# wavey-ai/soundkit

Measured on AMD Instinct MI355X. Metric: AAC-LC 1024-sample frames/s (whole node) + xrealtime, batch=4096 48 kHz stereo, higher is better.
Workload: dtype f32 (synthesis f32; s16 between the kernels as in the reference; FIR: the 16-bit samples as 2 x f16 exactly, the f32 taps as 2 x f16 to 2^-24, f32 accumulate; 1.0e-7 rel. RMS vs f64)

## Files before the change

soundkit_amd/csrc/aac_synth.hip:

```cpp
#include "sk_device.h"

#define SK_SYNTH_LOAD(p) (*(p))
#define SK_SYNTH_STORE(v, p) (*(p) = (v))

namespace sk {

namespace {

typedef float f2 __attribute__((ext_vector_type(2)));
typedef float f4 __attribute__((ext_vector_type(4)));

#ifndef SK_SYNTH_BLOCK_WAVES
#define SK_SYNTH_BLOCK_WAVES 4
#endif
constexpr int kWavesPerBlock = SK_SYNTH_BLOCK_WAVES;
#ifndef SK_WAVES_PER_SIMD
#define SK_WAVES_PER_SIMD 3
#endif
#ifndef SK_PREFETCH_DEPTH
#define SK_PREFETCH_DEPTH 1
#endif
constexpr int kDepth = SK_PREFETCH_DEPTH;
constexpr int kWavesPerSimd = SK_WAVES_PER_SIMD;
constexpr int kExchange = 576;
constexpr int kStage = 1024;

__device__ __forceinline__ f2 cmul(f2 a, f2 b) {
    return (f2){fmaf(a.x, b.x, -a.y * b.y), fmaf(a.x, b.y, a.y * b.x)};
}
__device__ __forceinline__ f2 cadd(f2 a, f2 b) { return (f2){a.x + b.x, a.y + b.y}; }
__device__ __forceinline__ f2 csub(f2 a, f2 b) { return (f2){a.x - b.x, a.y - b.y}; }
__device__ __forceinline__ f2 mul_mi(f2 a) { return (f2){a.y, -a.x}; }

__device__ __forceinline__ void dft8(f2 (&x)[8]) {
    const float h = 0.70710678118654752440f;
    f2 t0 = cadd(x[0], x[4]), t1 = csub(x[0], x[4]);
    f2 t2 = cadd(x[2], x[6]), t3 = mul_mi(csub(x[2], x[6]));
    f2 e0 = cadd(t0, t2), e2 = csub(t0, t2), e1 = cadd(t1, t3), e3 = csub(t1, t3);
    f2 u0 = cadd(x[1], x[5]), u1 = csub(x[1], x[5]);
    f2 u2 = cadd(x[3], x[7]), u3 = mul_mi(csub(x[3], x[7]));
    f2 o0 = cadd(u0, u2), o2 = csub(u0, u2), o1 = cadd(u1, u3), o3 = csub(u1, u3);
    f2 w1 = (f2){(o1.x + o1.y) * h, (o1.y - o1.x) * h};
    f2 w2 = mul_mi(o2);
    f2 w3 = (f2){(o3.y - o3.x) * h, -(o3.x + o3.y) * h};
    x[0] = cadd(e0, o0); x[4] = csub(e0, o0);
    x[1] = cadd(e1, w1); x[5] = csub(e1, w1);
    x[2] = cadd(e2, w2); x[6] = csub(e2, w2);
    x[3] = cadd(e3, w3); x[7] = csub(e3, w3);
}

__device__ __forceinline__ void wave_sync() {
    __builtin_amdgcn_fence(__ATOMIC_ACQ_REL, "wavefront");
    __builtin_amdgcn_wave_barrier();
}

typedef const __attribute__((address_space(4))) SynthEntry *const_entries;
__device__ __forceinline__ const_entries as_constant(const SynthEntry *p) {
    return reinterpret_cast<const_entries>(reinterpret_cast<uintptr_t>(p));
}

typedef uint32_t u2 __attribute__((ext_vector_type(2)));
__device__ __forceinline__ u2 pack4_s16(const f4 &v) {
    return (u2){dev_pack2_s16(v.x, v.y), dev_pack2_s16(v.z, v.w)};
}

__device__ __forceinline__ const float *first_half_window(const float *win, int seq, int prev_shape) {
    return seq == 3 ? win + 6656 + 1024 * prev_shape : win + 2048 * prev_shape;
}
__device__ __forceinline__ const float *second_half_window(const float *win, int seq, int shape) {
    return seq == 1 ? win + 4608 + 1024 * shape : win + 2048 * shape + 1024;
}

typedef __attribute__((address_space(3))) f2 lds_f2;
typedef __attribute__((address_space(3))) f4 lds_f4;
typedef __attribute__((address_space(3))) float lds_f;

__device__ __forceinline__ void read_positions(const lds_f *buf, int lane, float (&v)[16]) {
#pragma unroll
    for (int r = 0; r < 2; ++r) {
        const int j = 4 * lane + 256 * r;
        const f4 f = *reinterpret_cast<const lds_f4 *>(buf + j);
        const f4 m = *reinterpret_cast<const lds_f4 *>(buf + 1020 - j);
        v[8 * r + 0] = f.x; v[8 * r + 1] = f.y; v[8 * r + 2] = f.z; v[8 * r + 3] = f.w;
        v[8 * r + 4] = m.x; v[8 * r + 5] = m.y; v[8 * r + 6] = m.z; v[8 * r + 7] = m.w;
    }
}

__device__ __forceinline__ void write_positions(lds_f *buf, int lane, const float (&v)[16]) {
#pragma unroll
    for (int r = 0; r < 2; ++r) {
        const int j = 4 * lane + 256 * r;
        *reinterpret_cast<lds_f4 *>(buf + j) = (f4){v[8 * r + 0], v[8 * r + 1], v[8 * r + 2], v[8 * r + 3]};
        *reinterpret_cast<lds_f4 *>(buf + 1020 - j) = (f4){v[8 * r + 4], v[8 * r + 5], v[8 * r + 6], v[8 * r + 7]};
    }
}

__device__ __forceinline__ void fft512(f2 (&z)[8], lds_f2 *ex, const lds_f2 *t64, f2 base2, int lane) {
    const int hi3 = lane >> 3, lo3 = lane & 7;
    dft8(z);
#pragma unroll
    for (int k = 1; k < 8; ++k) z[k] = cmul(z[k], t64[8 * k + hi3]);
#pragma unroll
    for (int k = 0; k < 8; ++k) ex[k * 68 + lane] = z[k];
    wave_sync();
#pragma unroll
    for (int n2 = 0; n2 < 8; ++n2) z[n2] = cmul(ex[lo3 * 68 + 8 * n2 + hi3], base2);
    wave_sync();
    dft8(z);
#pragma unroll
    for (int k = 1; k < 8; ++k) z[k] = cmul(z[k], t64[8 * k + hi3]);
#pragma unroll
    for (int k = 0; k < 8; ++k) ex[hi3 * 72 + k * 8 + lo3] = z[k];
    wave_sync();
#pragma unroll
    for (int n3 = 0; n3 < 8; ++n3) z[n3] = ex[n3 * 72 + lane];
    wave_sync();
    dft8(z);
}

__device__ __attribute__((noinline)) void synth_rare_frame(lds_f2 *ex, lds_f *stage, const lds_f2 *tw_lds,
                                                            const lds_f2 *t64, float base2_re, float base2_im,
                                                            const lds_f *short_win, const lds_f2 *w64, const lds_f2 *tw_short,
                                                            float *out_ptr, int16_t *out16_ptr, int seq, int prev_shape,
                                                            int shape, int lane) {
    const int hi3 = lane >> 3, lo3 = lane & 7;
    (void)base2_re, (void)base2_im, (void)t64, (void)tw_lds, (void)seq;
    const lds_f *prev_short = short_win + 256 * prev_shape;
    const lds_f *cur_short = short_win + 256 * shape;
    f2 z[8];
#pragma unroll
    for (int r = 0; r < 8; ++r) z[r] = ex[64 * r + lane];
    float dly[16];
    read_positions(stage, lane, dly);
    wave_sync();
    float o[16], d[16];

    {
#pragma unroll
        for (int w = 0; w < 8; ++w) ex[64 * w + lane] = z[w];
        wave_sync();
#pragma unroll
        for (int b2 = 0; b2 < 8; ++b2) z[b2] = ex[64 * hi3 + lo3 + 8 * b2];
        wave_sync();
        dft8(z);
#pragma unroll
        for (int kb = 1; kb < 8; ++kb) z[kb] = cmul(z[kb], w64[lo3 * kb]);
#pragma unroll
        for (int kb = 0; kb < 8; ++kb) ex[64 * hi3 + 8 * kb + lo3] = z[kb];
        wave_sync();
#pragma unroll
        for (int aa = 0; aa < 8; ++aa) z[aa] = ex[64 * hi3 + 8 * lo3 + aa];
        wave_sync();
        dft8(z);
#pragma unroll
        for (int ka = 0; ka < 8; ++ka) {
            const int k = lo3 + 8 * ka;
            ex[64 * hi3 + k] = cmul(tw_short[k], (f2){z[ka].x, -z[ka].y});
        }
        wave_sync();
        const bool odd_lane = lane & 1;
        const int lo = odd_lane ? (63 - lane) >> 1 : lane >> 1;
        float cw[4], pw[2];
#pragma unroll
        for (int m = 0; m < 4; ++m) cw[m] = cur_short[lane + 64 * m];
        pw[0] = prev_short[lane];
        pw[1] = prev_short[lane + 64];
        float smp[8][4];
#pragma unroll
        for (int w = 0; w < 8; ++w) {
            const f2 A = ex[64 * w + lo], B = ex[64 * w + 32 + lo];
            const float s0 = odd_lane ? -A.y : -B.x, s1 = odd_lane ? B.x : A.y, s2 = odd_lane ? A.x : B.y, s3 = odd_lane ? B.y : A.x;
            smp[w][0] = s0 * (w == 0 ? pw[0] : cw[0]);
            smp[w][1] = s1 * (w == 0 ? pw[1] : cw[1]);
            smp[w][2] = s2 * cw[2];
            smp[w][3] = s3 * cw[3];
        }
        wave_sync();
#pragma unroll
        for (int half = 0; half < 2; ++half) {
#pragma unroll
            for (int r = 0; r < 4; ++r) *reinterpret_cast<lds_f4 *>(stage + 4 * lane + 256 * r) = (f4){0.f, 0.f, 0.f, 0.f};
            wave_sync();
#pragma unroll
            for (int parity = 0; parity < 2; ++parity) {
#pragma unroll
                for (int w = parity; w < 8; w += 2)
#pragma unroll
                    for (int m = 0; m < 4; ++m) {
                        const int base = 448 + 128 * w + 64 * m;
                        if ((base >> 10) != half) continue;
                        lds_f *at = stage + (base & 1023) + lane;
                        *at = *at + smp[w][m];
                    }
                wave_sync();
            }
            if (half == 0) read_positions(stage, lane, o);
            else read_positions(stage, lane, d);
            wave_sync();
        }
    }

    float pcm[16];
#pragma unroll
    for (int i = 0; i < 16; ++i) pcm[i] = o[i] + dly[i];
    write_positions((lds_f *)ex, lane, pcm);
    write_positions(stage, lane, d);
    wave_sync();
    (void)out_ptr, (void)out16_ptr;
}

template <bool OUT16, bool ONLY_LONG>
__global__ __launch_bounds__(kWavesPerBlock * 64, (ONLY_LONG && kDepth == 1) ? kWavesPerSimd + 1 : kWavesPerSimd) void k_aac_synth(SynthArgs a) {
    __shared__ f2 lds[kWavesPerBlock][kExchange];
    __shared__ float stage_lds[ONLY_LONG ? 1 : kWavesPerBlock][ONLY_LONG ? 4 : kStage];
    __shared__ f2 tw_tab[512];
    __shared__ f2 t64_tab[64];
    __shared__ float short_win_tab[ONLY_LONG ? 2 : 512];
    __shared__ f2 short_tw_tab[ONLY_LONG ? 1 : 128];

    const int lane = threadIdx.x & 63;
    const int wave = __builtin_amdgcn_readfirstlane(threadIdx.x >> 6);
    for (int i = threadIdx.x; i < 512; i += kWavesPerBlock * 64) tw_tab[i] = reinterpret_cast<const f2 *>(a.t.tw_long)[i];
    if (threadIdx.x < 64) t64_tab[threadIdx.x] = reinterpret_cast<const f2 *>(a.t.w64)[((threadIdx.x >> 3) * (threadIdx.x & 7)) & 63];
    if (!ONLY_LONG) {
        for (int i = threadIdx.x; i < 512; i += kWavesPerBlock * 64) short_win_tab[i] = a.t.win[4096 + i];
        if (threadIdx.x < 128)
            short_tw_tab[threadIdx.x] = threadIdx.x < 64 ? reinterpret_cast<const f2 *>(a.t.w64)[threadIdx.x] : reinterpret_cast<const f2 *>(a.t.tw_short)[threadIdx.x - 64];
    }
    __syncthreads();

    const uint32_t task_id = blockIdx.x * kWavesPerBlock + wave;
    if (task_id >= a.n_tasks) return;
    lds_f2 *ex = (lds_f2 *)lds[wave];
    lds_f *stage = (lds_f *)stage_lds[ONLY_LONG ? 0 : wave];
    const lds_f2 *tw_lds = (const lds_f2 *)tw_tab;
    const lds_f2 *t64 = (const lds_f2 *)t64_tab;

    const SynthTask task_v = a.tasks[task_id];
    const uint32_t count = __builtin_amdgcn_readfirstlane(task_v.count);
    const uint32_t state = __builtin_amdgcn_readfirstlane(task_v.state);
    if (count == 0) return;
    const const_entries entries = as_constant(a.entries + __builtin_amdgcn_readfirstlane(task_v.begin));

    const int hi3 = lane >> 3, lo3 = lane & 7;
    const f2 base2 = reinterpret_cast<const f2 *>(a.t.w512)[hi3 * lo3];

    float *delay_ptr = a.delay + (size_t)state * 1024;
    int prev_shape = __builtin_amdgcn_readfirstlane((int)a.prev_shape[state]);
    float dly[16];
    {
#pragma unroll
        for (int r = 0; r < 2; ++r) {
            const int j = 4 * lane + 256 * r;
            const f4 f = *reinterpret_cast<const f4 *>(delay_ptr + j);
            const f4 m = *reinterpret_cast<const f4 *>(delay_ptr + 1020 - j);
            dly[8 * r + 0] = f.x; dly[8 * r + 1] = f.y; dly[8 * r + 2] = f.z; dly[8 * r + 3] = f.w;
            dly[8 * r + 4] = m.x; dly[8 * r + 5] = m.y; dly[8 * r + 6] = m.z; dly[8 * r + 7] = m.w;
        }
    }

    auto load_spectrum = [&](f2 (&xin)[8], uint32_t e) {
        const float *src = a.coeffs + (size_t)__builtin_amdgcn_readfirstlane(entries[e].off1024) * 1024 + 2 * lane;
#pragma unroll
        for (int r = 0; r < 8; ++r) xin[r] = SK_SYNTH_LOAD(reinterpret_cast<const f2 *>(src + 128 * r));
    };
    auto frame = [&](f2 (&xin)[8], uint32_t e) __attribute__((always_inline)) {
        const uint32_t ent_off = entries[e].off1024, ent_win = entries[e].win;
        const uint32_t win = __builtin_amdgcn_readfirstlane(ent_win);
        const int seq = (int)(win & 3);
        const int shape = (win >> 2) & 1;
// ... 367 lines not shown
        }
        f4 f, m;
        f.x = -F0.x * W1f.x + dly[8 * r + 0]; f.y = -M1.y * W1f.y + dly[8 * r + 1];
        f.z = -F1.x * W1f.z + dly[8 * r + 2]; f.w = -M0.y * W1f.w + dly[8 * r + 3];
        m.x = M0.y * W1m.x + dly[8 * r + 4]; m.y = F1.x * W1m.y + dly[8 * r + 5];
        m.z = M1.y * W1m.z + dly[8 * r + 6]; m.w = F0.x * W1m.w + dly[8 * r + 7];
        if (OUT16) {
            SK_SYNTH_STORE(pack4_s16(f), reinterpret_cast<u2 *>(out16_ptr + j));
            SK_SYNTH_STORE(pack4_s16(m), reinterpret_cast<u2 *>(out16_ptr + 1020 - j));
        } else {
            SK_SYNTH_STORE(f, reinterpret_cast<f4 *>(out_ptr + j));
            SK_SYNTH_STORE(m, reinterpret_cast<f4 *>(out_ptr + 1020 - j));
        }
        dly[8 * r + 0] = F0.y * W2f.x; dly[8 * r + 1] = M1.x * W2f.y;
        dly[8 * r + 2] = F1.y * W2f.z; dly[8 * r + 3] = M0.x * W2f.w;
        dly[8 * r + 4] = M0.x * W2m.x; dly[8 * r + 5] = F1.y * W2m.y;
        dly[8 * r + 6] = M1.x * W2m.z; dly[8 * r + 7] = F0.y * W2m.w;
    };

    lds_f2 *stage = (lds_f2 *)stage_lds[WITH_SHORT ? wave : 0];
    auto store_pcm = [&](const float (&pcm)[16], uint32_t off) __attribute__((always_inline)) {
#pragma unroll
        for (int r = 0; r < 2; ++r) {
            const int j = 4 * lane + 256 * r;
            const f4 f = (f4){pcm[8 * r + 0], pcm[8 * r + 1], pcm[8 * r + 2], pcm[8 * r + 3]};
            const f4 m = (f4){pcm[8 * r + 4], pcm[8 * r + 5], pcm[8 * r + 6], pcm[8 * r + 7]};
            if (OUT16) {
                SK_SYNTH_STORE(pack4_s16(f), reinterpret_cast<u2 *>(a.pcm16 + (size_t)off * 1024 + j));
                SK_SYNTH_STORE(pack4_s16(m), reinterpret_cast<u2 *>(a.pcm16 + (size_t)off * 1024 + 1020 - j));
            } else {
                SK_SYNTH_STORE(f, reinterpret_cast<f4 *>(a.pcm + (size_t)off * 1024 + j));
                SK_SYNTH_STORE(m, reinterpret_cast<f4 *>(a.pcm + (size_t)off * 1024 + 1020 - j));
            }
        }
    };

    f2 xa[8], xb[8];
    load_spectrum(xa, ent_a, 0);
    load_spectrum(xb, ent_b, 0);
    for (uint32_t e = 0; e < count; ++e) {
        const uint32_t off_a = __builtin_amdgcn_readfirstlane(ent_a[e].off1024), off_b = __builtin_amdgcn_readfirstlane(ent_b[e].off1024);
        const uint32_t win_a = __builtin_amdgcn_readfirstlane(ent_a[e].win), win_b = __builtin_amdgcn_readfirstlane(ent_b[e].win);
        const int shape_a = (win_a >> 2) & 1, shape_b = (win_b >> 2) & 1;
        if constexpr (WITH_SHORT) {
            if ((win_a & 3u) == 2u) {
                {
                    const f2 tws = short_tw_tab[64 + lane];
                    const f2 tx = splat(tws.x), ty = splat(tws.y);
#pragma unroll
                    for (int w = 0; w < 8; ++w) {
                        const f2 even = (f2){xa[w].x, xb[w].x};
                        const f2 odd = (f2){-__shfl(xa[w].y, 63 - lane), -__shfl(xb[w].y, 63 - lane)};
                        const c2 zw = {odd * ty - even * tx, odd * tx + even * ty};
                        ex[64 * w + lane] = as_slot(zw);
                    }
                    f2 both[16];
#pragma unroll
                    for (int i = 0; i < 16; ++i) both[i] = (f2){dly_a[i], dly_b[i]};
                    write_positions2(stage, lane, both);
                    wave_sync();
                }
                synth_rare_pair(ex, stage, (const lds_f *)short_win_tab, (const lds_f2 *)short_tw_tab, (const lds_f2 *)short_tw_tab + 64, prev_a, shape_a, prev_b,
                                shape_b, lane);
                float pcm_a[16], pcm_b[16];
                {
                    f2 both[16];
                    read_positions2(stage, lane, both);
#pragma unroll
                    for (int i = 0; i < 16; ++i) {
                        dly_a[i] = both[i].x;
                        dly_b[i] = both[i].y;
                    }
                    read_positions2((const lds_f2 *)ex, lane, both);
#pragma unroll
                    for (int i = 0; i < 16; ++i) {
                        pcm_a[i] = both[i].x;
                        pcm_b[i] = both[i].y;
                    }
                    wave_sync();
                }
                const uint32_t ahead = e + 1 < count ? e + 1 : count - 1;
                load_spectrum(xa, ent_a, ahead);
                load_spectrum(xb, ent_b, ahead);
                store_pcm(pcm_a, off_a);
                store_pcm(pcm_b, off_b);
                prev_a = shape_a;
                prev_b = shape_b;
                continue;
            }
        }
        c2 z[8];
#pragma unroll
        for (int r = 0; r < 8; ++r) {
            const f2 even = (f2){xa[r].x, xb[r].x};
            const f2 odd = (f2){-__shfl(xa[7 - r].y, 63 - lane), -__shfl(xb[7 - r].y, 63 - lane)};
            const f2 t = tw_lds[lane + 64 * r];
            const f2 tx = splat(t.x), ty = splat(t.y);
            z[r] = {odd * ty - even * tx, odd * tx + even * ty};
        }
        Win wa, wb;
        int w1_a = 0, w2_a = 0, w1_b = 0, w2_b = 0;
        if constexpr (LDS_WIN) {
            const int seq_a = (int)(win_a & 3), seq_b = (int)(win_b & 3);
            w1_a = seq_a == 3 ? 6144 + 1024 * prev_a : 2048 * prev_a, w2_a = seq_a == 1 ? 4096 + 1024 * shape_a : 2048 * shape_a + 1024;
            w1_b = seq_b == 3 ? 6144 + 1024 * prev_b : 2048 * prev_b, w2_b = seq_b == 1 ? 4096 + 1024 * shape_b : 2048 * shape_b + 1024;
        } else {
            load_windows(wa, (int)(win_a & 3), prev_a, shape_a);
            load_windows(wb, (int)(win_b & 3), prev_b, shape_b);
        }
        {
            const uint32_t ahead = e + 1 < count ? e + 1 : count - 1;
            load_spectrum(xa, ent_a, ahead);
            load_spectrum(xb, ent_b, ahead);
        }
        fft512(z, ex, t64, base2, lane);
#pragma unroll
        for (int j = 0; j < 8; ++j) {
            const f2 t = tw_lds[lane + 64 * j];
            const f2 tx = splat(t.x), ty = splat(t.y);
            const c2 v = {fma2(tx, z[j].re, -(ty * -z[j].im)), fma2(tx, -z[j].im, ty * z[j].re)};
            ex[lane + 64 * j] = as_slot(v);
        }
        wave_sync();
        float *out_a = OUT16 ? nullptr : a.pcm + (size_t)off_a * 1024, *out_b = OUT16 ? nullptr : a.pcm + (size_t)off_b * 1024;
        int16_t *out16_a = OUT16 ? a.pcm16 + (size_t)off_a * 1024 : nullptr, *out16_b = OUT16 ? a.pcm16 + (size_t)off_b * 1024 : nullptr;
#pragma unroll
        for (int r = 0; r < 2; ++r) {
            const int q = 2 * lane + 128 * r;
            const f4 F0 = ex[256 + q], F1 = ex[257 + q], M0 = ex[254 - q], M1 = ex[255 - q];
            emit(r, (f2){F0.x, F0.z}, (f2){F1.x, F1.z}, (f2){M0.x, M0.z}, (f2){M1.x, M1.z}, wa, w1_a, w2_a, dly_a, out_a, out16_a);
            emit(r, (f2){F0.y, F0.w}, (f2){F1.y, F1.w}, (f2){M0.y, M0.w}, (f2){M1.y, M1.w}, wb, w1_b, w2_b, dly_b, out_b, out16_b);
        }
        wave_sync();
        prev_a = shape_a;
        prev_b = shape_b;
    }
    auto store_state = [&](float *p, const float (&d)[16]) {
#pragma unroll
        for (int r = 0; r < 2; ++r) {
            const int j = 4 * lane + 256 * r;
            *reinterpret_cast<f4 *>(p + j) = (f4){d[8 * r + 0], d[8 * r + 1], d[8 * r + 2], d[8 * r + 3]};
            *reinterpret_cast<f4 *>(p + 1020 - j) = (f4){d[8 * r + 4], d[8 * r + 5], d[8 * r + 6], d[8 * r + 7]};
        }
    };
    store_state(delay_a, dly_a);
    store_state(delay_b, dly_b);
    if (lane == 0) {
        a.prev_shape[state_a] = (uint8_t)prev_a;
        a.prev_shape[state_b] = (uint8_t)prev_b;
    }
}

constexpr int kTailRing = 2048;
constexpr int kTailDepth = 2;

__global__ __launch_bounds__(128, 2) void k_aac_tail(TailArgs ta) {
    const SynthArgs &a = ta.s;
    __shared__ f2 lds[2][kExchange];
    __shared__ f2 tw_tab[512];
    __shared__ f2 t64_tab[64];
    __shared__ __attribute__((aligned(16))) uint16_t ring_lds[2][2][kTailRing];
    __shared__ __attribute__((aligned(16))) uint32_t xchg[2][2][128];

    const int lane = threadIdx.x & 63;
    const int wave = __builtin_amdgcn_readfirstlane((int)(threadIdx.x >> 6));
    for (int i = threadIdx.x; i < 512; i += 128) tw_tab[i] = reinterpret_cast<const f2 *>(a.t.tw_long)[i];
    if (threadIdx.x < 64) t64_tab[threadIdx.x] = reinterpret_cast<const f2 *>(a.t.w64)[((threadIdx.x >> 3) * (threadIdx.x & 7)) & 63];
    for (int i = threadIdx.x; i < 2 * 2 * kTailRing / 8; i += 128) reinterpret_cast<sk_u32x4 *>(&ring_lds[0][0][0])[i] = (sk_u32x4){0u, 0u, 0u, 0u};
    __syncthreads();

    const uint32_t pair_id = blockIdx.x;
    lds_f2 *ex = (lds_f2 *)lds[wave];
    const lds_f2 *tw_lds = (const lds_f2 *)tw_tab;
    const lds_f2 *t64 = (const lds_f2 *)t64_tab;
    unsigned char *ring = reinterpret_cast<unsigned char *>(&ring_lds[wave][0][0]);

    const SynthTask task_v = a.tasks[2 * pair_id + (uint32_t)wave];
    const SynthTask other_v = a.tasks[2 * pair_id + (uint32_t)(wave ^ 1)];
    const uint32_t count = __builtin_amdgcn_readfirstlane(task_v.count);
    const uint32_t state = __builtin_amdgcn_readfirstlane(task_v.state);
    const uint32_t other_state = __builtin_amdgcn_readfirstlane(other_v.state);
    if (count == 0) return;
    const const_entries entries = as_constant(a.entries + __builtin_amdgcn_readfirstlane(task_v.begin));
    const bool stereo = (state ^ other_state) == 1u;
    const uint64_t first_elem = (uint64_t)__builtin_amdgcn_readfirstlane(entries[0].off1024) * 1024u;
    const uint32_t out_row = (uint32_t)(first_elem / ta.stream_stride);
    const uint32_t n_out = (1024u * count - 130u) / 3u;
    uint32_t *dst32 = reinterpret_cast<uint32_t *>(ta.out16 + (size_t)out_row * ta.out_stride * 2);
    int16_t *dst16 = ta.out16 + (size_t)out_row * ta.out_stride;

    const int hi3 = lane >> 3, lo3 = lane & 7;
    const f2 base2 = reinterpret_cast<const f2 *>(a.t.w512)[hi3 * lo3];

    sk_u32x4 af[10][2];
    {
        const sk_u32x4 *af_src = reinterpret_cast<const sk_u32x4 *>(ta.afrag_f16) + lane;
#pragma unroll
        for (int sidx = 0; sidx < 10; ++sidx)
#pragma unroll
            for (int k = 0; k < 2; ++k) af[sidx][k] = af_src[(sidx * 2 + k) * 64];
    }

    float *delay_ptr = a.delay + (size_t)state * 1024;
    int prev_shape = __builtin_amdgcn_readfirstlane((int)a.prev_shape[state]);
    float dly[16];
#pragma unroll
    for (int r = 0; r < 2; ++r) {
        const int j = 4 * lane + 256 * r;
        const f4 f = *reinterpret_cast<const f4 *>(delay_ptr + j);
        const f4 m = *reinterpret_cast<const f4 *>(delay_ptr + 1020 - j);
        dly[8 * r + 0] = f.x; dly[8 * r + 1] = f.y; dly[8 * r + 2] = f.z; dly[8 * r + 3] = f.w;
        dly[8 * r + 4] = m.x; dly[8 * r + 5] = m.y; dly[8 * r + 6] = m.z; dly[8 * r + 7] = m.w;
    }

    auto to_ring = [&](const f4 &v, int ring_pos) __attribute__((always_inline)) {
        const u2 p = pack4_s16(v);
        uint32_t p1a, p2a, p1b, p2b;
        dev_split_pair16_f16(p.x, p1a, p2a);
        dev_split_pair16_f16(p.y, p1b, p2b);
        *reinterpret_cast<u2 *>(ring + 2 * ring_pos) = (u2){p1a, p1b};
        *reinterpret_cast<u2 *>(ring + 2 * kTailRing + 2 * ring_pos) = (u2){p2a, p2b};
    };

    const int jq_off = 48 * (lane & 15) + 8 * (lane >> 4);
    auto fir_tile = [&](uint32_t T) __attribute__((always_inline)) {
        const int base = (int)(768u * T) - 128 + jq_off;
        sk_f32x4 acc = {0.f, 0.f, 0.f, 0.f};
#pragma unroll
        for (int sidx = 0; sidx < 10; ++sidx) {
            const int at = 2 * ((base + 32 * sidx) & (kTailRing - 1));
            const sk_u32x4 b1 = *reinterpret_cast<const sk_u32x4 *>(ring + at);
            acc = dev_mfma_f16(af[sidx][0], b1, acc);
            if (kFirProductsF16[sidx] == 3) {
                const sk_u32x4 b2 = *reinterpret_cast<const sk_u32x4 *>(ring + 2 * kTailRing + at);
                acc = dev_mfma_f16(af[sidx][1], b1, acc);
                acc = dev_mfma_f16(af[sidx][0], b2, acc);
            }
        }
        const uint32_t lo = dev_pack2_s16_scaled<31>(acc[0], acc[1]), hi = dev_pack2_s16_scaled<31>(acc[2], acc[3]);
        if (!stereo) {
            const uint32_t m0 = 256u * T + 16u * (uint32_t)(lane & 15) + 4u * (uint32_t)(lane >> 4);
            if (m0 + 3 < n_out) {
                *reinterpret_cast<u2 *>(dst16 + m0) = (u2){lo, hi};
            } else {
                if (m0 + 0 < n_out) dst16[m0 + 0] = (int16_t)(lo & 0xffffu);
                if (m0 + 1 < n_out) dst16[m0 + 1] = (int16_t)(lo >> 16);
                if (m0 + 2 < n_out) dst16[m0 + 2] = (int16_t)(hi & 0xffffu);
            }
            return;
        }
        uint32_t *mine = &xchg[T & 1u][wave][0];
        *reinterpret_cast<u2 *>(mine + 2 * lane) = (u2){lo, hi};
        __syncthreads();
        const uint32_t fm = 128u * (uint32_t)wave + 2u * (uint32_t)lane;
        const uint32_t word = 2u * (16u * ((fm >> 2) & 3u) + (fm >> 4)) + ((fm >> 1) & 1u);
        const uint32_t l2 = xchg[T & 1u][(state & 1u) ? (wave ^ 1) : wave][word];
        const uint32_t r2 = xchg[T & 1u][(state & 1u) ? wave : (wave ^ 1)][word];
        const uint32_t f0 = __builtin_amdgcn_perm(r2, l2, 0x05040100u), f1 = __builtin_amdgcn_perm(r2, l2, 0x07060302u);
        const uint32_t m0 = 256u * T + fm;
        if (m0 + 1 < n_out) *reinterpret_cast<u2 *>(dst32 + m0) = (u2){f0, f1};
        else if (m0 < n_out) dst32[m0] = f0;
    };

    auto load_spectrum = [&](f2 (&xin)[8], uint32_t e) {
        const float *src = a.coeffs + (size_t)__builtin_amdgcn_readfirstlane(entries[e].off1024) * 1024 + 2 * lane;
#pragma unroll
        for (int r = 0; r < 8; ++r) xin[r] = SK_SYNTH_LOAD(reinterpret_cast<const f2 *>(src + 128 * r));
    };

    uint32_t next_tile = 0;
    auto frame = [&](f2 (&xin)[8], uint32_t e) __attribute__((always_inline)) {
        const uint32_t win = __builtin_amdgcn_readfirstlane(entries[e].win);
        const int seq = (int)(win & 3);
        const int shape = (win >> 2) & 1;
        f2 z[8];
#pragma unroll
        for (int r = 0; r < 8; ++r) {
            const float even = xin[r].x;
            const float odd = -__shfl(xin[7 - r].y, 63 - lane);
            const f2 t = tw_lds[lane + 64 * r];
            z[r] = (f2){odd * t.y - even * t.x, odd * t.x + even * t.y};
        }
        const float *w1 = first_half_window(a.t.win, seq, prev_shape);
        const float *w2 = second_half_window(a.t.win, seq, shape);
        f4 w1f[2], w1m[2], w2f[2], w2m[2];
#pragma unroll
        for (int r = 0; r < 2; ++r) {
            const int j = 4 * lane + 256 * r;
            w1f[r] = *reinterpret_cast<const f4 *>(w1 + j);
            w1m[r] = *reinterpret_cast<const f4 *>(w1 + 1020 - j);
            w2f[r] = *reinterpret_cast<const f4 *>(w2 + j);
            w2m[r] = *reinterpret_cast<const f4 *>(w2 + 1020 - j);
        }
        load_spectrum(xin, e + kTailDepth < count ? e + kTailDepth : count - 1);
        fft512(z, ex, t64, base2, lane);
#pragma unroll
        for (int j = 0; j < 8; ++j) ex[lane + 64 * j] = cmul(tw_lds[lane + 64 * j], (f2){z[j].x, -z[j].y});
        wave_sync();
        const int frame_at = (int)((e & 1u) * 1024u);
#pragma unroll
        for (int r = 0; r < 2; ++r) {
            const int q = 2 * lane + 128 * r, j = 2 * q;
            const f4 F = *reinterpret_cast<const lds_f4 *>(&ex[256 + q]);
            const f4 M = *reinterpret_cast<const lds_f4 *>(&ex[254 - q]);
            const f4 W1f = w1f[r], W1m = w1m[r], W2f = w2f[r], W2m = w2m[r];
            f4 f, m;
            f.x = -F.x * W1f.x + dly[8 * r + 0]; f.y = -M.w * W1f.y + dly[8 * r + 1];
            f.z = -F.z * W1f.z + dly[8 * r + 2]; f.w = -M.y * W1f.w + dly[8 * r + 3];
            m.x = M.y * W1m.x + dly[8 * r + 4]; m.y = F.z * W1m.y + dly[8 * r + 5];
            m.z = M.w * W1m.z + dly[8 * r + 6]; m.w = F.x * W1m.w + dly[8 * r + 7];
            to_ring(f, frame_at + j);
            to_ring(m, frame_at + 1020 - j);
            dly[8 * r + 0] = F.y * W2f.x; dly[8 * r + 1] = M.z * W2f.y;
            dly[8 * r + 2] = F.w * W2f.z; dly[8 * r + 3] = M.x * W2f.w;
            dly[8 * r + 4] = M.x * W2m.x; dly[8 * r + 5] = F.w * W2m.y;
            dly[8 * r + 6] = M.z * W2m.z; dly[8 * r + 7] = F.y * W2m.w;
        }
        wave_sync();
        prev_shape = shape;
        const uint32_t have = 1024u * (e + 1);
        while (256u * next_tile < n_out && (768u * next_tile + 896u <= have || e + 1 == count)) {
            fir_tile(next_tile);
            ++next_tile;
        }
    };
    f2 ring_x[kTailDepth][8];
#pragma unroll
    for (int d = 0; d < kTailDepth; ++d) load_spectrum(ring_x[d], (uint32_t)d < count ? (uint32_t)d : count - 1);
    for (uint32_t e0 = 0; e0 < count; e0 += kTailDepth) {
#pragma unroll
        for (int d = 0; d < kTailDepth; ++d)
            if (e0 + (uint32_t)d < count) frame(ring_x[d], e0 + (uint32_t)d);
    }

#pragma unroll
    for (int r = 0; r < 2; ++r) {
        const int j = 4 * lane + 256 * r;
        *reinterpret_cast<f4 *>(delay_ptr + j) = (f4){dly[8 * r + 0], dly[8 * r + 1], dly[8 * r + 2], dly[8 * r + 3]};
        *reinterpret_cast<f4 *>(delay_ptr + 1020 - j) = (f4){dly[8 * r + 4], dly[8 * r + 5], dly[8 * r + 6], dly[8 * r + 7]};
    }
    if (lane == 0) a.prev_shape[state] = (uint8_t)prev_shape;
}

__device__ __forceinline__ int16_t float_sample_to_i16(float s) {
    return (int16_t)dev_float_sample_to_i16_f32(s);
}

__global__ __launch_bounds__(256) void k_frames_to_s16(const float *planar, int16_t *out, const FrameSpan *frames,
                                                       uint32_t n) {
    const uint32_t f = blockIdx.x;
    if (f >= n) return;
    const FrameSpan sp = frames[f];
    const float *src = planar + (size_t)sp.off1024 * 1024;
    int16_t *dst = out + (size_t)sp.off1024 * 1024;
    const int i = threadIdx.x * 4;
    if (sp.channels == 2) {
        const float4 l = *reinterpret_cast<const float4 *>(src + i);
        const float4 r = *reinterpret_cast<const float4 *>(src + 1024 + i);
        union { int16_t h[8]; uint4 v; } u;
        u.h[0] = float_sample_to_i16(l.x); u.h[1] = float_sample_to_i16(r.x);
        u.h[2] = float_sample_to_i16(l.y); u.h[3] = float_sample_to_i16(r.y);
        u.h[4] = float_sample_to_i16(l.z); u.h[5] = float_sample_to_i16(r.z);
        u.h[6] = float_sample_to_i16(l.w); u.h[7] = float_sample_to_i16(r.w);
        *reinterpret_cast<uint4 *>(dst + 2 * i) = u.v;
    } else {
        const float4 l = *reinterpret_cast<const float4 *>(src + i);
        union { int16_t h[4]; uint2 v; } u;
        u.h[0] = float_sample_to_i16(l.x); u.h[1] = float_sample_to_i16(l.y);
        u.h[2] = float_sample_to_i16(l.z); u.h[3] = float_sample_to_i16(l.w);
        *reinterpret_cast<uint2 *>(dst + i) = u.v;
    }
}

__global__ __launch_bounds__(256) void k_dequantize(const int16_t *q, const int16_t *sf, float *out, size_t n,
                                                    const float *pow43, const float *sftab) {
    size_t i = (size_t)blockIdx.x * blockDim.x + threadIdx.x;
    const size_t stride = (size_t)gridDim.x * blockDim.x;
    for (; i < n; i += stride) {
        const int v = q[i];
        const int s = sf[i];
        float r = 0.0f;
        if (v != 0) {
            const int mag = v < 0 ? -v : v;
            const float m = mag < 8192 ? pow43[mag] : powf((float)mag, 4.0f / 3.0f);
            const float sc = (s >= -256 && s <= 511) ? sftab[s + 256] : powf(2.0f, ((float)s - 100.0f) * 0.25f);
            r = (v < 0 ? -1.0f : 1.0f) * m * sc;
        }
        out[i] = r;
    }
}

__global__ __launch_bounds__(256) void k_reset_streams(float *delay, uint8_t *shape, uint32_t *pns, const uint32_t *ids) {
    const uint32_t id = ids[blockIdx.x];
    f4 *d = reinterpret_cast<f4 *>(delay + (size_t)id * 2048);
    d[threadIdx.x] = (f4){0.f, 0.f, 0.f, 0.f};
    d[threadIdx.x + 256] = (f4){0.f, 0.f, 0.f, 0.f};
    if (threadIdx.x < 2) shape[(size_t)id * 2 + threadIdx.x] = 0;
    if (threadIdx.x == 2) pns[id] = 0x1f2e3d4cu;
}

__global__ __launch_bounds__(256) void k_zero_spans(float *base, const uint32_t *ids, uint32_t span) {
    f4 *d = reinterpret_cast<f4 *>(base + (size_t)ids[blockIdx.x] * span);
    for (uint32_t i = threadIdx.x; i < span / 4; i += 256) d[i] = (f4){0.f, 0.f, 0.f, 0.f};
}

}

hipError_t launch_zero_spans(float *base, const uint32_t *ids, uint32_t n, uint32_t span_floats, hipStream_t s) {
    if (n == 0) return hipSuccess;
    if (span_floats % 4) return hipErrorInvalidValue;
    hipLaunchKernelGGL(k_zero_spans, dim3(n), dim3(256), 0, s, base, ids, span_floats);
    return hipGetLastError();
}

hipError_t launch_reset_streams(float *delay, uint8_t *shape, uint32_t *pns, const uint32_t *ids, uint32_t n, hipStream_t s) {
    if (n == 0) return hipSuccess;
    hipLaunchKernelGGL(k_reset_streams, dim3(n), dim3(256), 0, s, delay, shape, pns, ids);
    return hipGetLastError();
}

hipError_t launch_aac_synth(const SynthArgs &a, hipStream_t s) {
    if (a.n_tasks == 0) return hipSuccess;
    const uint32_t blocks = (a.n_tasks + kWavesPerBlock - 1) / kWavesPerBlock;
    if (a.only_long) {
        if (a.pcm16) hipLaunchKernelGGL((k_aac_synth<true, true>), dim3(blocks), dim3(kWavesPerBlock * 64), 0, s, a);
        else hipLaunchKernelGGL((k_aac_synth<false, true>), dim3(blocks), dim3(kWavesPerBlock * 64), 0, s, a);
    } else {
        if (a.pcm16) hipLaunchKernelGGL((k_aac_synth<true, false>), dim3(blocks), dim3(kWavesPerBlock * 64), 0, s, a);
        else hipLaunchKernelGGL((k_aac_synth<false, false>), dim3(blocks), dim3(kWavesPerBlock * 64), 0, s, a);
    }
    return hipGetLastError();
}

hipError_t launch_aac_synth_pairs(const SynthArgs &a, bool with_short, hipStream_t s) {
    if (a.n_tasks < 2) return hipSuccess;
    if (a.n_tasks & 1) return hipErrorInvalidValue;
    const uint32_t pairs = a.n_tasks / 2, blocks = (pairs + kWavesPerBlock - 1) / kWavesPerBlock;
    const dim3 grid(blocks), block(kWavesPerBlock * 64);
    if (with_short) {
        if (a.pcm16) hipLaunchKernelGGL((k_aac_synth_pair<true, true>), grid, block, 0, s, a);
        else hipLaunchKernelGGL((k_aac_synth_pair<false, true>), grid, block, 0, s, a);
    } else {
        if (a.pcm16) hipLaunchKernelGGL((k_aac_synth_pair<true, false>), grid, block, 0, s, a);
        else hipLaunchKernelGGL((k_aac_synth_pair<false, false>), grid, block, 0, s, a);
    }
    return hipGetLastError();
}

hipError_t launch_aac_tail(const TailArgs &ta, hipStream_t s) {
    if (ta.s.n_tasks < 2) return hipSuccess;
    if ((ta.s.n_tasks & 1) || !ta.afrag_f16 || !ta.out16 || ta.stream_stride == 0) return hipErrorInvalidValue;
    hipLaunchKernelGGL(k_aac_tail, dim3(ta.s.n_tasks / 2), dim3(128), 0, s, ta);
    return hipGetLastError();
}

hipError_t launch_frames_to_s16(const float *planar, int16_t *out, const FrameSpan *frames, uint32_t n, hipStream_t s) {
    if (n == 0) return hipSuccess;
    hipLaunchKernelGGL(k_frames_to_s16, dim3(n), dim3(256), 0, s, planar, out, frames, n);
    return hipGetLastError();
}

hipError_t launch_dequantize(const int16_t *q, const int16_t *sf, float *out, size_t n, const float *pow43,
                             const float *sftab, hipStream_t s) {
    if (n == 0) return hipSuccess;
    size_t blocks = (n + 255) / 256;
    if (blocks > 8192) blocks = 8192;
    hipLaunchKernelGGL(k_dequantize, dim3((unsigned)blocks), dim3(256), 0, s, q, sf, out, n, pow43, sftab);
    return hipGetLastError();
}

}
```

Baseline: 258.1 million.

## Interleave FIR MFMA chains into the synthesis FFT via scheduling points

The resampling FIR tiles, which used to run after each frame's IMDCT, are now deferred by one frame. Their MFMA steps and LDS reads are spread through the next frame's pre-twiddle, FFT512 and post-twiddle at fixed insertion points, with sched_barriers to pin placement. The goal is to overlap the matrix-core work with the VALU/LDS-bound FFT and hide latency inside one wave. The spectrum prefetch depth drops from 2 to 1, and a drain loop finishes the remaining tiles. The cost is more register pressure from holding the operands of two chains, plus rigid schedule constraints that may hurt the compiler's own scheduling.

```diff
diff --git a/soundkit_amd/csrc/aac_synth.hip b/soundkit_amd/csrc/aac_synth.hip
--- a/soundkit_amd/csrc/aac_synth.hip
+++ b/soundkit_amd/csrc/aac_synth.hip
@@ -1,4 +1,6 @@
 #include "sk_device.h"
+
+#include <type_traits>
 
 #define SK_SYNTH_LOAD(p) (*(p))
 #define SK_SYNTH_STORE(v, p) (*(p) = (v))
@@ -32,21 +34,33 @@
 __device__ __forceinline__ f2 csub(f2 a, f2 b) { return (f2){a.x - b.x, a.y - b.y}; }
 __device__ __forceinline__ f2 mul_mi(f2 a) { return (f2){a.y, -a.x}; }
 
-__device__ __forceinline__ void dft8(f2 (&x)[8]) {
+constexpr int kDftPoints = 7;
+template <class Point>
+__device__ __forceinline__ void dft8_points(f2 (&x)[8], Point &&point, int first) {
     const float h = 0.70710678118654752440f;
     f2 t0 = cadd(x[0], x[4]), t1 = csub(x[0], x[4]);
     f2 t2 = cadd(x[2], x[6]), t3 = mul_mi(csub(x[2], x[6]));
+    point(first + 0);
     f2 e0 = cadd(t0, t2), e2 = csub(t0, t2), e1 = cadd(t1, t3), e3 = csub(t1, t3);
+    point(first + 1);
     f2 u0 = cadd(x[1], x[5]), u1 = csub(x[1], x[5]);
     f2 u2 = cadd(x[3], x[7]), u3 = mul_mi(csub(x[3], x[7]));
+    point(first + 2);
     f2 o0 = cadd(u0, u2), o2 = csub(u0, u2), o1 = cadd(u1, u3), o3 = csub(u1, u3);
+    point(first + 3);
     f2 w1 = (f2){(o1.x + o1.y) * h, (o1.y - o1.x) * h};
     f2 w2 = mul_mi(o2);
     f2 w3 = (f2){(o3.y - o3.x) * h, -(o3.x + o3.y) * h};
+    point(first + 4);
     x[0] = cadd(e0, o0); x[4] = csub(e0, o0);
     x[1] = cadd(e1, w1); x[5] = csub(e1, w1);
+    point(first + 5);
     x[2] = cadd(e2, w2); x[6] = csub(e2, w2);
     x[3] = cadd(e3, w3); x[7] = csub(e3, w3);
+    point(first + 6);
+}
+__device__ __forceinline__ void dft8(f2 (&x)[8]) {
+    dft8_points(x, [](int) {}, 0);
 }
 
 __device__ __forceinline__ void wave_sync() {
@@ -116,6 +130,47 @@
     for (int n3 = 0; n3 < 8; ++n3) z[n3] = ex[n3 * 72 + lane];
     wave_sync();
     dft8(z);
+}
+
+constexpr int kFftPoints = 3 * kDftPoints + 3 * 4;
+template <class Point>
+__device__ __forceinline__ void fft512_points(f2 (&z)[8], lds_f2 *ex, const lds_f2 *t64, f2 base2, int lane, Point &&point, int first) {
+    const int hi3 = lane >> 3, lo3 = lane & 7;
+    f2 w[8];
+    dft8_points(z, point, first);
+#pragma unroll
+    for (int k = 1; k < 8; ++k) w[k] = t64[8 * k + hi3];
+#pragma unroll
+    for (int k = 1; k < 8; ++k) {
+        z[k] = cmul(z[k], w[k]);
+        if (k & 1) point(first + kDftPoints + k / 2);
+    }
+#pragma unroll
+    for (int k = 0; k < 8; ++k) ex[k * 68 + lane] = z[k];
+    wave_sync();
+#pragma unroll
+    for (int n2 = 0; n2 < 8; ++n2) w[n2] = ex[lo3 * 68 + 8 * n2 + hi3];
+    wave_sync();
+#pragma unroll
+    for (int n2 = 0; n2 < 8; ++n2) {
+        z[n2] = cmul(w[n2], base2);
+        if (n2 & 1) point(first + kDftPoints + 4 + n2 / 2);
+    }
+    dft8_points(z, point, first + kDftPoints + 8);
+#pragma unroll
+    for (int k = 1; k < 8; ++k) w[k] = t64[8 * k + hi3];
+#pragma unroll
+    for (int k = 1; k < 8; ++k) {
+        z[k] = cmul(z[k], w[k]);
+        if (k & 1) point(first + 2 * kDftPoints + 8 + k / 2);
+    }
+#pragma unroll
+    for (int k = 0; k < 8; ++k) ex[hi3 * 72 + k * 8 + lo3] = z[k];
+    wave_sync();
+#pragma unroll
+    for (int n3 = 0; n3 < 8; ++n3) z[n3] = ex[n3 * 72 + lane];
+    wave_sync();
+    dft8_points(z, point, first + 2 * kDftPoints + 12);
 }
 
 __device__ __attribute__((noinline)) void synth_rare_frame(lds_f2 *ex, lds_f *stage, const lds_f2 *tw_lds,
@@ -789,7 +844,18 @@
 }
 
 constexpr int kTailRing = 2048;
-constexpr int kTailDepth = 2;
+constexpr int kTailDepth = 1;
+constexpr int kTailSteps = 24;
+constexpr int tail_step_window(int k) { return k == 0 ? 0 : k < 22 ? 1 + (k - 1) / 3 : k - 14; }
+constexpr int tail_step_product(int k) { return k == 0 || k >= 22 ? 0 : (k - 1) % 3; }
+constexpr bool tail_steps_match_products() {
+    int k = 0;
+    for (int sidx = 0; sidx < 10; ++sidx)
+        for (int prod = 0; prod < kFirProductsF16[sidx]; ++prod, ++k)
+            if (k >= kTailSteps || tail_step_window(k) != sidx || tail_step_product(k) != prod) return false;
+    return k == kTailSteps;
+}
+static_assert(tail_steps_match_products(), "tail_step_window / tail_step_product restate kFirProductsF16");
 
 __global__ __launch_bounds__(128, 2) void k_aac_tail(TailArgs ta) {
     const SynthArgs &a = ta.s;
@@ -860,20 +926,31 @@
     };
 
     const int jq_off = 48 * (lane & 15) + 8 * (lane >> 4);
-    auto fir_tile = [&](uint32_t T) __attribute__((always_inline)) {
-        const int base = (int)(768u * T) - 128 + jq_off;
-        sk_f32x4 acc = {0.f, 0.f, 0.f, 0.f};
-#pragma unroll
-        for (int sidx = 0; sidx < 10; ++sidx) {
-            const int at = 2 * ((base + 32 * sidx) & (kTailRing - 1));
-            const sk_u32x4 b1 = *reinterpret_cast<const sk_u32x4 *>(ring + at);
-            acc = dev_mfma_f16(af[sidx][0], b1, acc);
-            if (kFirProductsF16[sidx] == 3) {
-                const sk_u32x4 b2 = *reinterpret_cast<const sk_u32x4 *>(ring + 2 * kTailRing + at);
-                acc = dev_mfma_f16(af[sidx][1], b1, acc);
-                acc = dev_mfma_f16(af[sidx][0], b2, acc);
-            }
-        }
+    struct Chain {
+        sk_f32x4 acc;
+        sk_u32x4 b[10][2];
+        int base2;
+    };
+    auto chain_read = [&](Chain &c, int sidx) __attribute__((always_inline)) {
+        const int at = (c.base2 + 64 * sidx) & (2 * kTailRing - 1);
+        c.b[sidx][0] = *reinterpret_cast<const sk_u32x4 *>(ring + at);
+        if (kFirProductsF16[sidx] == 3) c.b[sidx][1] = *reinterpret_cast<const sk_u32x4 *>(ring + 2 * kTailRing + at);
+    };
+    auto chain_begin = [&](Chain &c, uint32_t T) __attribute__((always_inline)) {
+        c.acc = (sk_f32x4){0.f, 0.f, 0.f, 0.f};
+        c.base2 = 2 * ((int)(768u * T) - 128 + jq_off);
+        chain_read(c, 0);
+        chain_read(c, 1);
+    };
+    auto chain_step = [&](Chain &c, int k) __attribute__((always_inline)) {
+        const int sidx = tail_step_window(k), prod = tail_step_product(k);
+        if (prod == 0) {
+            if (sidx >= 1 && sidx <= 6) chain_read(c, sidx + 1);
+            if (sidx == 7) { chain_read(c, 8); chain_read(c, 9); }
+        }
+        c.acc = dev_mfma_f16(af[sidx][prod == 1 ? 1 : 0], c.b[sidx][prod == 2 ? 1 : 0], c.acc);
+    };
+    auto tile_store = [&](uint32_t T, const sk_f32x4 &acc) __attribute__((always_inline)) {
         const uint32_t lo = dev_pack2_s16_scaled<31>(acc[0], acc[1]), hi = dev_pack2_s16_scaled<31>(acc[2], acc[3]);
         if (!stereo) {
             const uint32_t m0 = 256u * T + 16u * (uint32_t)(lane & 15) + 4u * (uint32_t)(lane >> 4);
@@ -905,36 +982,73 @@
         for (int r = 0; r < 8; ++r) xin[r] = SK_SYNTH_LOAD(reinterpret_cast<const f2 *>(src + 128 * r));
     };
 
-    uint32_t next_tile = 0;
-    auto frame = [&](f2 (&xin)[8], uint32_t e) __attribute__((always_inline)) {
+    uint32_t next_tile = 0, pend_n = 0;
+    auto frame = [&](auto np_tag, f2 (&xin)[8], uint32_t e) __attribute__((always_inline)) {
+        constexpr int NP = decltype(np_tag)::value;
+        constexpr int kPoints = 8 + kFftPoints + 8;
+        static_assert(kPoints >= 2 * kTailSteps, "every step of two chains needs an insertion point");
+        constexpr int kWindowPoint = 8 + 2 * kDftPoints + 12;
         const uint32_t win = __builtin_amdgcn_readfirstlane(entries[e].win);
         const int seq = (int)(win & 3);
         const int shape = (win >> 2) & 1;
-        f2 z[8];
-#pragma unroll
-        for (int r = 0; r < 8; ++r) {
-            const float even = xin[r].x;
-            const float odd = -__shfl(xin[7 - r].y, 63 - lane);
-            const f2 t = tw_lds[lane + 64 * r];
-            z[r] = (f2){odd * t.y - even * t.x, odd * t.x + even * t.y};
-        }
+        Chain c0, c1;
+        chain_begin(c0, next_tile);
         const float *w1 = first_half_window(a.t.win, seq, prev_shape);
         const float *w2 = second_half_window(a.t.win, seq, shape);
         f4 w1f[2], w1m[2], w2f[2], w2m[2];
-#pragma unroll
-        for (int r = 0; r < 2; ++r) {
+        auto load_windows = [&](int r) __attribute__((always_inline)) {
             const int j = 4 * lane + 256 * r;
             w1f[r] = *reinterpret_cast<const f4 *>(w1 + j);
             w1m[r] = *reinterpret_cast<const f4 *>(w1 + 1020 - j);
             w2f[r] = *reinterpret_cast<const f4 *>(w2 + j);
             w2m[r] = *reinterpret_cast<const f4 *>(w2 + 1020 - j);
+        };
+        auto point = [&](int i) __attribute__((always_inline)) {
+            if (i == kWindowPoint) {
+                __builtin_amdgcn_sched_barrier(0);
+                load_windows(0);
+            }
+            const int k = NP == 2 ? i : (i & 1) ? -1 : i / 2;
+            if (k < 0 || k >= NP * kTailSteps) return;
+            __builtin_amdgcn_sched_barrier(0);
+            if (NP == 2 && k == kTailSteps - 3) chain_begin(c1, next_tile + 1);
+            if (k < kTailSteps) chain_step(c0, k);
+            else chain_step(c1, k - kTailSteps);
+            __builtin_amdgcn_sched_barrier(0);
+        };
+        f2 z[8];
+        {
+            float odd[8];
+            f2 t[8];
+#pragma unroll
+            for (int r = 0; r < 8; ++r) {
+                odd[r] = -__shfl(xin[7 - r].y, 63 - lane);
+                t[r] = tw_lds[lane + 64 * r];
+            }
+#pragma unroll
+            for (int r = 0; r < 8; ++r) {
+                const float even = xin[r].x;
+                z[r] = (f2){odd[r] * t[r].y - even * t[r].x, odd[r] * t[r].x + even * t[r].y};
+                point(r);
+            }
         }
         load_spectrum(xin, e + kTailDepth < count ? e + kTailDepth : count - 1);
-        fft512(z, ex, t64, base2, lane);
-#pragma unroll
-        for (int j = 0; j < 8; ++j) ex[lane + 64 * j] = cmul(tw_lds[lane + 64 * j], (f2){z[j].x, -z[j].y});
+        fft512_points(z, ex, t64, base2, lane, point, 8);
+        {
+            f2 t[8];
+#pragma unroll
+            for (int j = 0; j < 8; ++j) t[j] = tw_lds[lane + 64 * j];
+#pragma unroll
+            for (int j = 0; j < 8; ++j) {
+                ex[lane + 64 * j] = cmul(t[j], (f2){z[j].x, -z[j].y});
+                point(8 + kFftPoints + j);
+            }
+        }
         wave_sync();
+        if (NP == 2 || pend_n) tile_store(next_tile, c0.acc);
+        if constexpr (NP == 2) tile_store(next_tile + 1, c1.acc);
         const int frame_at = (int)((e & 1u) * 1024u);
+        load_windows(1);
 #pragma unroll
         for (int r = 0; r < 2; ++r) {
             const int q = 2 * lane + 128 * r, j = 2 * q;
@@ -955,11 +1069,14 @@
         }
         wave_sync();
         prev_shape = shape;
+    };
+    auto run_frame = [&](f2 (&xin)[8], uint32_t e) __attribute__((always_inline)) {
+        if (pend_n == 2) frame(std::integral_constant<int, 2>{}, xin, e);
+        else frame(std::integral_constant<int, 1>{}, xin, e);
+        next_tile += pend_n;
         const uint32_t have = 1024u * (e + 1);
-        while (256u * next_tile < n_out && (768u * next_tile + 896u <= have || e + 1 == count)) {
-            fir_tile(next_tile);
-            ++next_tile;
-        }
+        pend_n = 0;
+        while (pend_n < 2 && 256u * (next_tile + pend_n) < n_out && 768u * (next_tile + pend_n) + 896u <= have) ++pend_n;
     };
     f2 ring_x[kTailDepth][8];
 #pragma unroll
@@ -967,7 +1084,14 @@
     for (uint32_t e0 = 0; e0 < count; e0 += kTailDepth) {
 #pragma unroll
         for (int d = 0; d < kTailDepth; ++d)
-            if (e0 + (uint32_t)d < count) frame(ring_x[d], e0 + (uint32_t)d);
+            if (e0 + (uint32_t)d < count) run_frame(ring_x[d], e0 + (uint32_t)d);
+    }
+    for (; 256u * next_tile < n_out; ++next_tile) {
+        Chain c;
+        chain_begin(c, next_tile);
+#pragma unroll
+        for (int k = 0; k < kTailSteps; ++k) chain_step(c, k);
+        tile_store(next_tile, c.acc);
     }
 
 #pragma unroll
```

Result: no change. 257.1 million, median of 3 (-0.4%).
